# BICLab/Spike2Former

Measured on AMD Instinct MI355X. Metric: fwd+bwd images/sec, 512x512 T=4 ADE20K-150, higher is better.
Workload: dtype f32 (fp32-equivalent: bf16 hi+mid+lo split operands on bf16 MFMA, fp32 accumulate; spike maps stored as bf16, exact); 1 GPU; C2: 512x512 T=4 K=150 Meta-SpikeFormer [64, 128, 256, 360] + MaskFormer head, per-GPU batch 2; global_batch=2, parallelism=dp1, weights=random-init (name-seeded)

## Files before the change

include/s2f.h:

```cpp
#ifndef S2F_H
#define S2F_H

#include <stdint.h>

#ifdef __cplusplus
extern "C" {
#endif

#define S2F_OK 0
#define S2F_EINVAL (-1)
#define S2F_EALIGN (-2)
#define S2F_ELAUNCH (-3)

#define S2F_ABI_VERSION 52
#define S2F_STAT_SLOTS 256

int s2f_version(void);
const char* s2f_last_error(void);

void* s2f_event_create(void);
void s2f_event_destroy(void* event);
int s2f_time_next_call(void* start_event, void* stop_event);
int s2f_event_elapsed_us(void* start_event, void* stop_event, double* microseconds);

int64_t s2f_lif_mask_words(int64_t n);

int s2f_lif_fwd(const float* x, const float* v_in, void* y, float* v_out, uint64_t* mask, uint8_t* count_u8,
                uint64_t* stats, int64_t n, float vth, int D, int y_bf16, void* stream);

int s2f_lif_bwd(const float* gy, const float* gv_out, const uint64_t* mask, float* gx, int64_t n, float vth, int D,
                void* stream);
int s2f_lif_bwd_ports(const float* gy, const float* gy2, const float* gv_out, const uint64_t* mask, const float* skip, float* gx,
                      int64_t n, float vth, int D, void* stream);

int s2f_lif_leaky_fwd(const float* x, const float* v_in, void* y, float* v_out, uint64_t* mask, uint64_t* stats, int64_t n, float vth,
                      int D, float tau, int decay_input, int y_bf16, void* stream);
int s2f_lif_leaky_bwd(const float* gy, const float* gv_out, const uint64_t* mask, float* gx, float* gv_in, int64_t n, float vth, int D,
                      float tau, int decay_input, void* stream);

int s2f_sum2_lif_fwd(const float* x, const float* e, const float* pos, void* y_key, void* y_value, uint64_t* mask_key,
                     uint64_t* mask_value, int64_t TB, int64_t B, int64_t C, int64_t L, float vth, int D, int y_bf16,
                     void* stream);
int s2f_sum2_lif_bwd(const float* g_key, const float* g_value, const uint64_t* mask_key, const uint64_t* mask_value,
                     float* gx, int64_t n, int D, void* stream);
int s2f_sum2_lif_bwd_ex(const float* g_key, const float* g_value, const uint64_t* mask_key, const uint64_t* mask_value, float* gx,
                        float* gx_key, int64_t n, int D, void* stream);
int s2f_sum2_lif_bwd_ports(const float* g_key, const float* g_key2, const float* g_value, const float* g_value2,
// ... 136 lines not shown
                           float* bn_partials, int batch, int Mo, int Ki, int N, void* stream);
int s2f_bn_partials_finalize(const float* partials, int64_t P, const float* conv_bias, double* sums_out, int64_t N, int64_t C,
                             int64_t L, void* stream);
int s2f_bn_grouped_ok(int64_t N, int64_t C, int64_t L);
int s2f_bn_act_fwd_grouped(const float* z, const float* conv_bias, float* stat_out, float* running_mean, float* running_var,
                           const float* gamma, const float* beta, float* u_out, void* y_out, uint64_t* mask, int groups, int64_t N,
                           int64_t C, int64_t L, float momentum, float eps, float vth, int D, int y_bf16, void* stream);
int s2f_bn_act_bwd_grouped(const float* z, const float* conv_bias, const float* stat, const float* gamma, const float* g_u,
                           const float* g_y, const uint64_t* mask, float* gz, float* dgamma, float* dbeta, int groups, int64_t N,
                           int64_t C, int64_t L, float vth, int D, void* stream);
int s2f_bn_bwd_ports_ok(int64_t N, int64_t C, int64_t L, int training, int D);
int s2f_bn_act_bwd_ports(const float* z, const float* conv_bias, const float* stat, const float* gamma, const float* g_u,
                         const float* g_y, const float* g_y2, const float* g_v, const uint64_t* mask, double* sums_zeroed, float* gz,
                         float* g_residual, float* dgamma, float* dbeta, int64_t N, int64_t C, int64_t L, int training, float vth,
                         int D, void* stream);

int s2f_bn_act_bwd_split(const float* z, const float* conv_bias, const float* stat, const float* gamma, const float* g_u,
                         const float* g_y, const float* g_v, const uint64_t* mask, double* sums_zeroed, uint16_t* gz_split,
                         float* g_residual, float* dgamma, float* dbeta, int64_t N, int64_t C, int64_t L, int training,
                         float vth, int D, void* stream);
int s2f_pgemm_dx_split(const uint16_t* w_pack, const uint16_t* G_split, int64_t plane_stride, float* DX, int batch, int Mo,
                       int Ki, int N, int cfg, void* stream);
int s2f_spike_gemm_dw_bf16_split(const uint16_t* dY_split, int64_t plane_stride, const uint16_t* X, float* dW, int batch, int M,
                                 int K, int L, int accumulate, void* stream);
int s2f_spike_gemm_dw_grouped_split(const int64_t* jobs, int njobs, int bkv, void* stream);
int s2f_gemm_dw_general(const float* dY, int64_t dy_batch_stride, const float* X, int64_t x_batch_stride, float* dW, int batch,
                        int M, int K, int L, int accumulate, void* stream);
int s2f_gemm_dw_general_grouped(const int64_t* jobs, int njobs, void* stream);

int s2f_upsample2x_fwd(const float* x, float* y, int64_t planes, int h, int w, void* stream);
int s2f_upsample2x_sigmoid_fwd(const float* x, float* y, int64_t planes, int h, int w, void* stream);
int s2f_upsample2x_bwd(const float* gy, float* gx, int64_t planes, int h, int w, void* stream);
int s2f_upsample2x_bwd_add(const float* gy, const float* add, float* gx, int64_t planes, int h, int w, void* stream);

#define S2F_RESIZE_ALIGN_CORNERS 1
#define S2F_RESIZE_SIGMOID 2
#define S2F_RESIZE_FLIP_H 4
#define S2F_RESIZE_FLIP_V 8
int s2f_resize_fwd(const float* x, float* y, int64_t planes, int64_t plane_stride, int row_stride, int row0, int col0, int h, int w,
                   int H, int W, int flags, void* stream);
int s2f_resize_bwd_add(const float* gy, const float* add, float* gx, int64_t planes, int h, int w, int H, int W, int flags,
                       void* stream);
int s2f_seg_argmax(const float* x, int64_t* label, float* label_f, int K, int64_t HW, int sigmoid, float threshold, void* stream);
int s2f_seg_label(const float* x, int64_t* label, float* label_f, int K, int64_t plane_stride, int row_stride, int row0, int col0,
                  int h, int w, int H, int W, int flags, float threshold, void* stream);
int s2f_tta_accumulate(const float* x, float* acc, int K, int64_t plane_stride, int row_stride, int row0, int col0, int h, int w,
                       int H, int W, int flags, int first, void* stream);
int s2f_tta_finish(float* acc, int64_t* label, float* label_f, int K, int64_t HW, int n_views, float threshold, void* stream);

int s2f_slide_windows(const float* x, float* out, int B, int C, int H, int W, int crop_h, int crop_w, int stride_h, int stride_w,
                      int w0, int n, void* stream);
int s2f_slide_accumulate(const float* logits, float* preds, int B, int K, int H, int W, int crop_h, int crop_w, int stride_h,
                         int stride_w, int w0, int n, void* stream);

#define S2F_SEG_HIST_MAX_CLASSES 2048
#define S2F_SEG_PRED_I64 0
#define S2F_SEG_PRED_F32 1
#define S2F_SEG_LABEL_U8 0
#define S2F_SEG_LABEL_I64 1
#define S2F_SEG_REDUCE_ZERO_LABEL 1
int s2f_seg_hist(const void* pred, int pred_dtype, const void* label, int label_dtype, int64_t label_row_stride,
                 int64_t label_pixel_stride, int W, int64_t HW, int K, int ignore_index, int flags, int64_t* totals, void* stream);
#define S2F_SEG_CONF_LDS_BYTES 131072
#define S2F_SEG_CONF_GLOBAL 2
int s2f_seg_confusion(const void* pred, int pred_dtype, const void* label, int label_dtype, int64_t label_row_stride,
                      int64_t label_pixel_stride, int W, int64_t HW, int K, int ignore_index, int flags, int64_t* matrix, void* stream);
// ... 163 lines not shown
```

spike2former_amd/_lib.py:

```python
import ctypes
import os

import torch

_HERE = os.path.dirname(os.path.abspath(__file__))
LIB_PATH = os.environ.get("S2F_LIB") or os.path.join(_HERE, "libs2f_hip.so")

_p, _i, _i64, _f = ctypes.c_void_p, ctypes.c_int, ctypes.c_int64, ctypes.c_float

SIGNATURES = {
    "s2f_version": (_i, []),
    "s2f_last_error": (ctypes.c_char_p, []),
    "s2f_event_create": (_p, []),
    "s2f_event_destroy": (None, [_p]),
    "s2f_time_next_call": (_i, [_p, _p]),
    "s2f_event_elapsed_us": (_i, [_p, _p, ctypes.POINTER(ctypes.c_double)]),
    "s2f_lif_mask_words": (_i64, [_i64]),
    "s2f_lif_fwd": (_i, [_p, _p, _p, _p, _p, _p, _p, _i64, _f, _i, _i, _p]),
    "s2f_lif_bwd": (_i, [_p, _p, _p, _p, _i64, _f, _i, _p]),
    "s2f_lif_bwd_ports": (_i, [_p] * 6 + [_i64, _f, _i, _p]),
    "s2f_lif_leaky_fwd": (_i, [_p, _p, _p, _p, _p, _p, _i64, _f, _i, _f, _i, _i, _p]),
    "s2f_lif_leaky_bwd": (_i, [_p, _p, _p, _p, _p, _i64, _f, _i, _f, _i, _p]),
    "s2f_sum2_lif_fwd": (_i, [_p] * 7 + [_i64] * 4 + [_f, _i, _i, _p]),
    "s2f_sum2_lif_bwd": (_i, [_p] * 5 + [_i64, _i, _p]),
    "s2f_sum2_lif_bwd_ex": (_i, [_p] * 6 + [_i64, _i, _p]),
    "s2f_sum2_lif_bwd_ports": (_i, [_p] * 9 + [_i64, _i, _p]),
    "s2f_mask_loss_fwd": (_i, [_p] * 4 + [_i64, _i, _i, _f, _f, _p]),
    "s2f_mask_loss_bwd": (_i, [_p] * 5 + [_i64, _i, _i, _f, _f, _p]),
    "s2f_scale_affine_fwd": (_i, [_p] * 5 + [_i, _p]),
    "s2f_scale_affine_bwd": (_i, [_p] * 8 + [_i, _p]),
    "s2f_lif_seq_fwd": (_i, [_p, _p, _p, _p, _p, _p, _i, _i64, _f, _i, _p]),
    "s2f_lif_seq_bwd": (_i, [_p, _p, _p, _p, _p, _i, _i64, _f, _i, _p]),
    "s2f_bn_single_pass": (_i, [_i64] * 3),
    "s2f_bn_mask_words": (_i64, [_i64] * 3),
    "s2f_bn2_fused_ok": (_i, [_i64] * 3),
    "s2f_bn2_act_fwd": (_i, [_p] * 8 + [_f, _f] + [_p] * 5 + [_f, _f] + [_p] * 7 + [_i64] * 3 + [_f, _i, _i, _p]),
    "s2f_bn2_act_bwd": (_i, [_p] * 5 + [_f] + [_p] * 10 + [_i64] * 3 + [_f, _i, _p]),
    "s2f_bn_stats": (_i, [_p] * 3 + [_i64] * 3 + [_p]),
    "s2f_bn_act_fwd": (_i, [_p] * 16 + [_i64] * 3 + [_f, _f, _i, _f, _i, _i, _p]),
    "s2f_bn_act_bwd": (_i, [_p] * 13 + [_i64] * 3 + [_i, _f, _i, _p]),
    "s2f_bn_up_ok": (_i, [_i64] * 4 + [_i, _i]),
    "s2f_bn_act_up_fwd": (_i, [_p] * 16 + [_i64] * 4 + [_f, _f, _i, _f, _i, _i, _p]),
    "s2f_im2col": (_i, [_p, _p] + [_i] * 9 + [_p]),
    "s2f_col2im": (_i, [_p, _p] + [_i] * 8 + [_p]),
    "s2f_dwconv_fwd": (_i, [_p] * 4 + [_i] * 7 + [_p]),
    "s2f_dwconv_stats_slots": (_i64, [_i] * 3),
    "s2f_dwconv_fwd_stats": (_i, [_p] * 4 + [_i64] + [_i] * 5 + [_p]),
    "s2f_dwconv_bn_lif_fwd": (_i, [_p] * 7 + [_f] + [_p] * 3 + [_i] * 7 + [_f, _i, _p]),
    "s2f_dwconv_bwd_input": (_i, [_p] * 3 + [_i] * 6 + [_p]),
    "s2f_dwconv_bwd_weight": (_i, [_p] * 4 + [_i] * 8 + [_p]),
    "s2f_split_bf16x3": (_i, [_p, _p, _i, _i, _i, _i, _p]),
    "s2f_split_bf16x3_multi": (_i, [_p, _i, _i64, _p]),
    "s2f_spike_gemm_fwd": (_i, [_p] * 4 + [_i] * 7 + [_p]),
    "s2f_upsample2x_fwd": (_i, [_p, _p, _i64, _i, _i, _p]),
    "s2f_upsample2x_sigmoid_fwd": (_i, [_p, _p, _i64, _i, _i, _p]),
    "s2f_upsample2x_bwd": (_i, [_p, _p, _i64, _i, _i, _p]),
    "s2f_upsample2x_bwd_add": (_i, [_p, _p, _p, _i64, _i, _i, _p]),
    "s2f_resize_fwd": (_i, [_p, _p, _i64, _i64] + [_i] * 8 + [_p]),
    "s2f_resize_bwd_add": (_i, [_p, _p, _p, _i64] + [_i] * 5 + [_p]),
    "s2f_seg_argmax": (_i, [_p, _p, _p, _i, _i64, _i, _f, _p]),
    "s2f_seg_label": (_i, [_p, _p, _p, _i, _i64] + [_i] * 8 + [_f, _p]),
    "s2f_tta_accumulate": (_i, [_p, _p, _i, _i64] + [_i] * 9 + [_p]),
    "s2f_tta_finish": (_i, [_p, _p, _p, _i, _i64, _i, _f, _p]),
    "s2f_slide_windows": (_i, [_p, _p] + [_i] * 10 + [_p]),
    "s2f_slide_accumulate": (_i, [_p, _p] + [_i] * 10 + [_p]),
    "s2f_seg_hist": (_i, [_p, _i, _p, _i, _i64, _i64, _i, _i64, _i, _i, _i, _p, _p]),
    "s2f_seg_confusion": (_i, [_p, _i, _p, _i, _i64, _i64, _i, _i64, _i, _i, _i, _p, _p]),
    "s2f_seg_draw": (_i, [_p, _p, _i, _p, _i, _p, _i, ctypes.c_double, _i, _i, _i, _p, _p]),
    "s2f_aug_param_bytes": (_i, []),
    "s2f_aug_crop_stats": (_i, [_p, _i64, _p, _i, _i, _i, _i, _i, ctypes.c_double, _p, _p]),
    "s2f_aug_apply": (_i, [_p, _i64, _p, _p, _i, _i, _i] + [_f] * 6 + [_i, _f, _i, _i, _p, _p, _p]),
    "s2f_view_param_bytes": (_i, []),
    "s2f_test_views": (_i, [_p, _i64, _p, _i, _i, _i] + [_f] * 6 + [_i, _f, _p, _i64, _p]),
    "s2f_transpose_last2": (_i, [_p, _p, _i64, _i, _i, _p]),
    "s2f_transpose_last2_add": (_i, [_p, _p, _p, _i64, _i, _i, _p]),
    "s2f_sum_n": (_i, [_p, _i, _p, _i64, _p]),
    "s2f_transpose_scale_add_fwd": (_i, [_p, _p, _p, _p, _i64, _i, _i, _p]),
    "s2f_transpose_scale_add_bwd": (_i, [_p, _p, _p, _p, _p, _i64, _i, _i, _p]),
    "s2f_spike_conv3x3_fwd": (_i, [_p, _p, _p, _p] + [_i] * 8 + [_p]),
    "s2f_spike_conv3x3_dw": (_i, [_p, _p, _p] + [_i] * 6 + [_p]),
    "s2f_conv3x3_general": (_i, [_p, _p, _p] + [_i] * 7 + [_p]),
    "s2f_split_gemm": (_i, [_p, _i64, _i64, _i, _p, _i64, _i, _i64, _i, _p, _i64, _f, _i, _i, _i, _i, _i, _i, _p]),
    "s2f_spike_gemm_dw": (_i, [_p, _p, _p, _i, _i, _i, _i, _i, _i, _p]),
    "s2f_to_bf16_exact": (_i, [_p, _p, _i64, _p]),
    "s2f_spike_gemm_fwd_bf16": (_i, [_p] * 4 + [_i] * 7 + [_p]),
    "s2f_spike_conv3x3_fwd_bf16": (_i, [_p, _p, _p, _p] + [_i] * 8 + [_p]),
    "s2f_spike_gemm_dw_bf16": (_i, [_p, _p, _p, _i, _i, _i, _i, _i, _p]),
    "s2f_spike_gemm_fwd_bf16_ex": (_i, [_p, _i64, _p, _i64, _i, _i64, _p, _i64, _f, _p, _i, _i, _i, _i, _i, _i, _p]),
    "s2f_pgemm_nn_bf16_ex": (_i, [_p, _i64, _p, _i64, _i, _i64, _p, _i64, _f, _p, _i, _i, _i, _i, _p]),
    "s2f_spike_gemm_dw_grouped": (_i, [_p, _i, _i, _p]),
# ... 111 lines not shown
```

spike2former_amd/csrc/im2col.hip:

```cpp
#include "s2f_common.h"

namespace {

template <typename T>
struct Vec4;
template <>
struct Vec4<float> {
  typedef float4 type;
};
template <>
struct Vec4<unsigned short> {
  typedef uint2 type;
};

template <typename T, int S>
__global__ __launch_bounds__(256) void im2col_kernel(const T* __restrict__ x, T* __restrict__ cols, int C, int H, int W, int kh,
                                                     int kw, int stride_rt, int pad, int Ho, int Wo) {
  const int stride = S > 0 ? S : stride_rt;
  const int L = Ho * Wo, l0 = ((int)blockIdx.x * 256 + (int)threadIdx.x) * 4;
  if (l0 >= L) return;
  const int rowi = blockIdx.y, kk = kh * kw;
  const int c = rowi / kk, tap = rowi - c * kk;
  const int ky = tap / kw, kx = tap - ky * kw;
  const T* xp = x + ((int64_t)blockIdx.z * C + c) * (int64_t)H * W;
  T v[4];
  int oy = l0 / Wo, ox = l0 - oy * Wo;
#pragma unroll
  for (int o = 0; o < 4; ++o) {
    const int iy = oy * stride + ky - pad, ix = ox * stride + kx - pad;
    v[o] = (l0 + o < L && iy >= 0 && iy < H && ix >= 0 && ix < W) ? xp[(int64_t)iy * W + ix] : (T)0;
    if (++ox == Wo) ox = 0, ++oy;
  }
  T* cp = cols + ((int64_t)blockIdx.z * gridDim.y + rowi) * (int64_t)L + l0;
  if ((L & 3) == 0) {
    typename Vec4<T>::type pk;
    __builtin_memcpy(&pk, v, sizeof(pk));
    *reinterpret_cast<typename Vec4<T>::type*>(cp) = pk;
  } else {
#pragma unroll
    for (int o = 0; o < 4; ++o)
      if (l0 + o < L) cp[o] = v[o];
  }
}

template <int S>
__global__ __launch_bounds__(256) void col2im_kernel(const float* __restrict__ cols, float* __restrict__ gx, int64_t planes, int H,
                                                     int W, int kh, int kw, int stride_rt, int pad, int Ho, int Wo) {
  const int stride = S > 0 ? S : stride_rt;
  const int kk = kh * kw, W4 = (W + 3) >> 2;
  const int64_t L = (int64_t)Ho * Wo;
  const int cell = (int)blockIdx.x * 256 + (int)threadIdx.x;
  const int64_t nc = (int64_t)blockIdx.z * gridDim.y + blockIdx.y;
  if (cell >= H * W4 || nc >= planes) return;
  const int y = cell / W4, x0 = (cell - y * W4) * 4;
  const float* cp = cols + nc * kk * L;
  float acc[4] = {0.f, 0.f, 0.f, 0.f};
  for (int ky = 0; ky < kh; ++ky) {
    const int ty = y + pad - ky;
    if (ty < 0) break;
    const int oy = ty / stride;
    if (oy * stride != ty || oy >= Ho) continue;
    for (int kx = 0; kx < kw; ++kx) {
      const float* rowp = cp + (int64_t)(ky * kw + kx) * L + (int64_t)oy * Wo;
#pragma unroll
      for (int o = 0; o < 4; ++o) {
        const int tx = x0 + o + pad - kx;
        const int ox = tx / stride;
        if (tx >= 0 && ox * stride == tx && ox < Wo && x0 + o < W) acc[o] += rowp[ox];
      }
    }
  }
  float* gp = gx + (nc * H + y) * (int64_t)W + x0;
  if ((W & 3) == 0) {
    *reinterpret_cast<float4*>(gp) = make_float4(acc[0], acc[1], acc[2], acc[3]);
  } else {
#pragma unroll
// ... 1 lines not shown
      if (x0 + o < W) gp[o] = acc[o];
  }
}

int geometry(const char* who, int N, int C, int H, int W, int kh, int kw, int stride, int pad, int& Ho, int& Wo) {
  S2F_REQUIRE(N > 0 && C > 0 && H > 0 && W > 0 && kh > 0 && kw > 0 && stride > 0 && pad >= 0, S2F_EINVAL, "%s: bad geometry", who);
  Ho = (H + 2 * pad - kh) / stride + 1;
  Wo = (W + 2 * pad - kw) / stride + 1;
  S2F_REQUIRE(Ho > 0 && Wo > 0, S2F_EINVAL, "%s: empty output", who);
  S2F_REQUIRE((int64_t)C * kh * kw < 65536 && N < 65536 && (int64_t)N * C < ((int64_t)1 << 30) && (int64_t)H * W < ((int64_t)1 << 31) &&
                  (int64_t)Ho * Wo < ((int64_t)1 << 31),
              S2F_EINVAL, "%s: shape too large for the launch grid", who);
  return S2F_OK;
}

constexpr int kStrides[] = {1, 2, 0};
template <class F>
void for_stride(int stride, const F& launch) {
  s2f_dispatch<kStrides>([&](int sv) { return sv == stride || sv == 0; }, launch);
}

}

extern "C" int s2f_im2col(const void* x, void* cols, int N, int C, int H, int W, int kh, int kw, int stride, int pad, int x_bf16,
                          void* stream) {
  S2F_REQUIRE(x && cols, S2F_EINVAL, "s2f_im2col: null pointer");
  int Ho, Wo;
  int rc = geometry("s2f_im2col", N, C, H, W, kh, kw, stride, pad, Ho, Wo);
  if (rc) return rc;
  S2F_REQUIRE((((int64_t)Ho * Wo) & 3) != 0 || (reinterpret_cast<uintptr_t>(cols) & (x_bf16 ? 7u : 15u)) == 0, S2F_EALIGN,
              "s2f_im2col: cols must be 8-byte (bf16) / 16-byte (fp32) aligned");
  const dim3 grid((unsigned)((((int64_t)Ho * Wo + 3) / 4 + 255) / 256), (unsigned)(C * kh * kw), (unsigned)N);
  hipStream_t s = (hipStream_t)stream;
  for_stride(stride, [&](auto i) {
    s2f_dispatch_bool(x_bf16 != 0, [&](auto bf) {
      using T = std::conditional_t<bf.value, unsigned short, float>;
      hipLaunchKernelGGL((im2col_kernel<T, kStrides[i]>), grid, dim3(256), 0, s, reinterpret_cast<const T*>(x),
                         reinterpret_cast<T*>(cols), C, H, W, kh, kw, stride, pad, Ho, Wo);
    });
  });
  return s2f_check_launch("s2f_im2col");
}

extern "C" int s2f_col2im(const float* cols, float* gx, int N, int C, int H, int W, int kh, int kw, int stride, int pad,
                          void* stream) {
  S2F_REQUIRE(cols && gx, S2F_EINVAL, "s2f_col2im: null pointer");
  int Ho, Wo;
  int rc = geometry("s2f_col2im", N, C, H, W, kh, kw, stride, pad, Ho, Wo);
  if (rc) return rc;
  S2F_REQUIRE((W & 3) != 0 || s2f_aligned16(gx), S2F_EALIGN, "s2f_col2im: gx must be 16-byte aligned");
  const int64_t planes = (int64_t)N * C;
  const unsigned gy = (unsigned)(planes < 32768 ? planes : 32768);
  const dim3 grid((unsigned)(((int64_t)H * ((W + 3) / 4) + 255) / 256), gy, (unsigned)((planes + gy - 1) / gy));
  hipStream_t s = (hipStream_t)stream;
  for_stride(stride, [&](auto i) {
    hipLaunchKernelGGL(col2im_kernel<kStrides[i]>, grid, dim3(256), 0, s, cols, gx, planes, H, W, kh, kw, stride, pad, Ho, Wo);
  });
  return s2f_check_launch("s2f_col2im");
}
```

spike2former_amd/csrc/upsample.hip:

```cpp
#include "s2f_common.h"

#pragma clang fp contract(off)

namespace {

__device__ __forceinline__ void taps(int o, int in_size, int& i0, int& i1, float& l1) {
  float src = ((float)o + 0.5f) * 0.5f - 0.5f;
  if (src < 0.f) src = 0.f;
  i0 = (int)src;
  i1 = i0 + (i0 < in_size - 1 ? 1 : 0);
  l1 = src - (float)i0;
}

__global__ __launch_bounds__(256) void up2x_fwd_kernel(const float* __restrict__ x, float* __restrict__ y, int64_t planes,
                                                       int h, int w) {
  const int W = 2 * w, H = 2 * h;
  const int64_t quads_per_row = W / 4;
  const int64_t total = planes * H * quads_per_row;
  for (int64_t idx = (int64_t)blockIdx.x * blockDim.x + threadIdx.x; idx < total; idx += (int64_t)gridDim.x * blockDim.x) {
    const int q = (int)(idx % quads_per_row);
    const int64_t r = idx / quads_per_row;
    const int oy = (int)(r % H);
    const int64_t p = r / H;
    int y0, y1;
// ... 140 lines not shown
    const float wfirst = ix0 == 0 ? 1.f : 0.75f, wlast = ix0 + 4 == w ? 1.f : 0.75f;
    float acc0[4] = {0.f, 0.f, 0.f, 0.f}, acc1[4] = {0.f, 0.f, 0.f, 0.f};
#pragma unroll
    for (int rr = 0; rr < 6; ++rr) {
      const int oy = 2 * iy - 1 + rr;
      if (oy < 0 || oy >= H) continue;
      const float* row = base + (int64_t)oy * W + 8 * k;
      const float4 a = *reinterpret_cast<const float4*>(row), b = *reinterpret_cast<const float4*>(row + 4);
      const float left = k > 0 ? row[-1] : 0.f, right = k + 1 < qw ? row[8] : 0.f;
      float hx[4];
      hx[0] = (0.25f * left + wfirst * a.x) + (0.75f * a.y + 0.25f * a.z);
      hx[1] = (0.25f * a.y + 0.75f * a.z) + (0.75f * a.w + 0.25f * b.x);
      hx[2] = (0.25f * a.w + 0.75f * b.x) + (0.75f * b.y + 0.25f * b.z);
      hx[3] = (0.25f * b.y + 0.75f * b.z) + (wlast * b.w + 0.25f * right);
      float w0 = 0.f, w1 = 0.f;
      if (rr <= 3) w0 = (rr == 0 || rr == 3) ? 0.25f : ((rr == 1 && iy == 0) ? 1.f : 0.75f);
      if (rr >= 2) w1 = (rr == 2 || rr == 5) ? 0.25f : ((rr == 4 && iy + 2 == h) ? 1.f : 0.75f);
#pragma unroll
      for (int i = 0; i < 4; ++i) {
        acc0[i] += w0 * hx[i];
        acc1[i] += w1 * hx[i];
      }
    }
    float* o = gx + (p * h + iy) * w + ix0;
    if (add) {
      const float* q = add + (p * h + iy) * w + ix0;
      const float4 a0 = *reinterpret_cast<const float4*>(q), a1 = *reinterpret_cast<const float4*>(q + w);
      acc0[0] += a0.x, acc0[1] += a0.y, acc0[2] += a0.z, acc0[3] += a0.w;
      acc1[0] += a1.x, acc1[1] += a1.y, acc1[2] += a1.z, acc1[3] += a1.w;
    }
    *reinterpret_cast<float4*>(o) = make_float4(acc0[0], acc0[1], acc0[2], acc0[3]);
    *reinterpret_cast<float4*>(o + w) = make_float4(acc1[0], acc1[1], acc1[2], acc1[3]);
  }
}

struct MaskPix {
  float s, t, bce, pt, at;
};

__device__ __forceinline__ MaskPix mask_pix(float u, unsigned char tb, float alpha) {
  MaskPix m;
  m.t = tb ? 1.f : 0.f;
  const float e = __expf(-fabsf(u));
  const float inv = 1.f / (1.f + e);
  m.s = u >= 0.f ? inv : e * inv;
  m.bce = fmaxf(u, 0.f) - u * m.t + log1pf(e);
  m.pt = (1.f - m.s) * m.t + m.s * (1.f - m.t);
  m.at = alpha * m.t + (1.f - alpha) * (1.f - m.t);
  return m;
}

__global__ __launch_bounds__(256) void mask_loss_fwd_kernel(const float* __restrict__ pred, const unsigned char* __restrict__ tgt,
                                                            const int64_t* __restrict__ gt, float* __restrict__ sums, int h,
                                                            int w, float alpha, float gamma, int chunks) {
  const int W = 2 * w, H = 2 * h;
  const int p = blockIdx.y;
  const float* pp = pred + (int64_t)p * h * w;
  const unsigned char* tp = tgt + gt[p] * (int64_t)H * W;
  const int quads = W / 4;
  const int64_t total = (int64_t)H * quads;
  const int64_t per = (total + chunks - 1) / chunks;
  const int64_t beg = blockIdx.x * per, end = beg + per < total ? beg + per : total;
  float a = 0.f, b = 0.f, c = 0.f, f = 0.f;
  for (int64_t idx = beg + threadIdx.x; idx < end; idx += 256) {
    const int q = (int)(idx % quads), oy = (int)(idx / quads);
    int y0, y1;
// ... 90 lines not shown
  if ((w & 3) == 0 && s2f_aligned16(x))
    hipLaunchKernelGGL(up2x_fwd_block_kernel<false>, plane_grid((int64_t)h * (w / 4), planes), dim3(256), 0, (hipStream_t)stream, x, y,
                       planes, h, w);
  else
    hipLaunchKernelGGL(up2x_fwd_kernel, dim3(grid_for(planes * 2 * h * (2 * w / 4))), dim3(256), 0, (hipStream_t)stream, x, y,
                       planes, h, w);
  return s2f_check_launch("s2f_upsample2x_fwd");
}

extern "C" int s2f_upsample2x_sigmoid_fwd(const float* x, float* y, int64_t planes, int h, int w, void* stream) {
  S2F_REQUIRE(x && y, S2F_EINVAL, "s2f_upsample2x_sigmoid_fwd: null pointer");
  S2F_REQUIRE(planes > 0 && h > 0 && w > 0 && (w % 4) == 0, S2F_EINVAL, "s2f_upsample2x_sigmoid_fwd: needs w %% 4 == 0");
  S2F_REQUIRE(s2f_aligned16(x) && s2f_aligned16(y), S2F_EALIGN, "s2f_upsample2x_sigmoid_fwd: 16-byte alignment");
  hipLaunchKernelGGL(up2x_fwd_block_kernel<true>, plane_grid((int64_t)h * (w / 4), planes), dim3(256), 0, (hipStream_t)stream, x, y,
                     planes, h, w);
  return s2f_check_launch("s2f_upsample2x_sigmoid_fwd");
}

extern "C" int s2f_upsample2x_bwd_add(const float* gy, const float* add, float* gx, int64_t planes, int h, int w, void* stream) {
  S2F_REQUIRE(gy && gx, S2F_EINVAL, "s2f_upsample2x_bwd: null pointer");
  S2F_REQUIRE(planes > 0 && h > 0 && w > 0, S2F_EINVAL, "s2f_upsample2x_bwd: bad shape");
  if ((w & 3) == 0 && (h & 1) == 0 && s2f_aligned16(gy) && s2f_aligned16(gx) && s2f_aligned16(add))
    hipLaunchKernelGGL(up2x_bwd_block_kernel, plane_grid((int64_t)(h / 2) * (w / 4), planes), dim3(256), 0, (hipStream_t)stream,
                       gy, gx, planes, h, w, add);
  else
    hipLaunchKernelGGL(up2x_bwd_kernel, dim3(grid_for(planes * h * w)), dim3(256), 0, (hipStream_t)stream, gy, gx, planes, h, w, add);
  return s2f_check_launch("s2f_upsample2x_bwd");
}

extern "C" int s2f_upsample2x_bwd(const float* gy, float* gx, int64_t planes, int h, int w, void* stream) {
  return s2f_upsample2x_bwd_add(gy, nullptr, gx, planes, h, w, stream);
}

extern "C" int s2f_mask_loss_fwd(const float* pred, const uint8_t* tgt, const int64_t* gt_index, float* sums, int64_t P, int h,
                                 int w, float alpha, float gamma, void* stream) {
  if (P == 0) return S2F_OK;
  S2F_REQUIRE(pred && tgt && gt_index && sums, S2F_EINVAL, "s2f_mask_loss_fwd: null pointer");
  S2F_REQUIRE(P > 0 && P < 65536 && h > 0 && w > 0 && (w % 2) == 0, S2F_EINVAL, "s2f_mask_loss_fwd: need 0 < P < 65536, even w");
  S2F_REQUIRE((reinterpret_cast<uintptr_t>(tgt) & 3u) == 0, S2F_EALIGN, "s2f_mask_loss_fwd: targets must be 4-byte aligned");
  hipStream_t s = (hipStream_t)stream;
  if (s2f_zero_async(sums, sizeof(float) * 4 * (size_t)P, s) != S2F_OK) return s2f_check_launch("s2f_mask_loss_fwd memset");
  const int64_t total = (int64_t)2 * h * (2 * w / 4);
  int chunks = (int)((total + 256 * 8 - 1) / (256 * 8));
  if (chunks < 1) chunks = 1;
  hipLaunchKernelGGL(mask_loss_fwd_kernel, dim3(chunks, (unsigned)P), dim3(256), 0, s, pred, tgt, gt_index, sums, h, w, alpha,
                     gamma, chunks);
  return s2f_check_launch("s2f_mask_loss_fwd");
}

extern "C" int s2f_mask_loss_bwd(const float* pred, const uint8_t* tgt, const int64_t* gt_index, const float* g_sums, float* gup,
                                 int64_t P, int h, int w, float alpha, float gamma, void* stream) {
  if (P == 0) return S2F_OK;
  S2F_REQUIRE(pred && tgt && gt_index && g_sums && gup, S2F_EINVAL, "s2f_mask_loss_bwd: null pointer");
  S2F_REQUIRE(P > 0 && P < 65536 && h > 0 && w > 0 && (w % 2) == 0, S2F_EINVAL, "s2f_mask_loss_bwd: need 0 < P < 65536, even w");
  S2F_REQUIRE((reinterpret_cast<uintptr_t>(tgt) & 3u) == 0 && s2f_aligned16(gup), S2F_EALIGN,
              "s2f_mask_loss_bwd: targets 4-byte, gradient 16-byte aligned");
  const int64_t total = (int64_t)2 * h * (2 * w / 4);
  int chunks = (int)((total + 256 * 4 - 1) / (256 * 4));
  if (chunks < 1) chunks = 1;
  hipLaunchKernelGGL(mask_loss_bwd_kernel, dim3(chunks, (unsigned)P), dim3(256), 0, (hipStream_t)stream, pred, tgt, gt_index,
                     g_sums, gup, h, w, alpha, gamma, chunks);
  return s2f_check_launch("s2f_mask_loss_bwd");
}
```

spike2former_amd/ops/bn.py:

```python
import torch

from .config import cfg
from .core import *
from .resize import upsample_bilinear


class _BNAct(torch.autograd.Function):

    @staticmethod
    def forward(ctx, z, conv_bias, gamma, beta, residual, v_in, running_mean, running_var, nbt, training, momentum,
                eps, lif_on, want_pre, keep_v, D, vth, stats, bf16, partials=None, up_lo=None, up_skip=False, groups=1):
        _need_cuda(z, conv_bias, gamma, beta, residual, v_in, up_lo)
        ctx.groups = groups
        if groups > 1:
            return _BNAct._forward_siblings(ctx, z, conv_bias, gamma, beta, running_mean, running_var, momentum, eps, lif_on, want_pre,
                                            D, vth, bf16, groups, plain=(residual is None and v_in is None and nbt is None and training
                                                                         and not keep_v and stats is None and up_lo is None))
        up_in = up_lo
        z = z.contiguous()
        N, C = z.shape[0], z.shape[1]
        L = z.numel() // (N * C)
        dev = z.device
        stat = torch.empty(3 * C, dtype=torch.float32, device=dev)
        s = _stream()
# ... 91 lines not shown
        outs = [t if t is not None else z.new_empty(0) for t in (u, y, None)]
        ctx.mark_non_differentiable(border, ydata, tok2, through, *[o for o, t in zip(outs, (u, y, None)) if t is None])
        return tuple(outs) + (border, ydata, tok2, through)

    @staticmethod
    def backward(ctx, g_u, g_y, g_v, g_border, _g_ydata, g_y2, g_through=None):
        z, conv_bias, gamma, stat, mask = ctx.saved_tensors
        N, C, L, training, D, vth, has_res, has_bias = ctx.cfg

        def prep(g):
            return None if (g is None or g.numel() == 0) else g.contiguous()
        g_u, g_y, g_v, g_y2 = prep(g_u), prep(g_y), prep(g_v), prep(g_y2)
        if ctx.groups > 1:
            if g_u is None and g_y is None:
                return (None,) * 23
            G = ctx.groups
            gz = torch.empty_like(z)
            dgamma = torch.empty(G * C, dtype=torch.float32, device=z.device)
            dbeta = torch.empty(G * C, dtype=torch.float32, device=z.device)
            alg = 4 * z.numel() * (2 + (g_u is not None) + (g_y is not None))
            _time_next("bn_lif_bwd" if g_y is not None else "bn_bwd", alg)
            check(lib.s2f_bn_act_bwd_grouped(_ptr(z), _ptr(conv_bias), _ptr(stat), _ptr(gamma), _ptr(g_u), _ptr(g_y), _ptr(mask),
                                             _ptr(gz), _ptr(dgamma), _ptr(dbeta), G, N, C, L, vth, D, _stream()),
                  "s2f_bn_act_bwd_grouped")
            return (gz, None, dgamma, dbeta) + (None,) * 19
        if g_y is None:
            g_y, g_y2 = g_y2, None
        if g_y2 is not None and not lib.s2f_bn_bwd_ports_ok(N, C, L, int(training), D):
            g_y, g_y2 = g_y + g_y2, None
        if g_u is None and g_y is None and g_v is None:
            return (None,) * 20 + (g_through, None, None)
        dev = z.device
        gz = torch.empty_like(z)
        g_res = torch.empty_like(z) if ((has_res and ctx.needs_input_grad[4]) or (ctx.up is not None and ctx.needs_input_grad[20])) else None
        dgamma = torch.empty(C, dtype=torch.float32, device=dev)
        dbeta = torch.empty(C, dtype=torch.float32, device=dev)
        ws = None if (training and lib.s2f_bn_single_pass(N, C, L)) else _take_zeroed(2 * C, dev)
        alg = 4 * z.numel() * (2 + (g_u is not None) + (g_y is not None) + (g_res is not None))
        _time_next("bn_lif_bwd" if g_y is not None else "bn_bwd", alg, moved=alg + 4 * z.numel() * (g_y2 is not None))
        check(lib.s2f_bn_act_bwd_ports(_ptr(z), _ptr(conv_bias), _ptr(stat), _ptr(gamma), _ptr(g_u), _ptr(g_y), _ptr(g_y2), _ptr(g_v),
                                       _ptr(mask), _ptr(ws), _ptr(gz), _ptr(g_res), _ptr(dgamma), _ptr(dbeta), N, C, L,
                                       int(training), vth, D, _stream()), "s2f_bn_act_bwd_ports")
        g_bias = None
        if has_bias:
            g_bias = None if training else gamma * stat[C:2 * C] * dbeta
        if ctx.needs_input_grad[5]:
            raise RuntimeError("gradient w.r.t. the incoming membrane is not supported by the fused BN+LIF op")
        if ctx.up is not None:
            g_lo = g_through
            if g_res is not None:
                h, w = ctx.up
                g_lo = torch.empty(N, C, h, w, dtype=torch.float32, device=dev)
                check(lib.s2f_upsample2x_bwd_add(_ptr(g_res), _ptr(None if g_through is None else g_through.contiguous()), _ptr(g_lo),
                                                 N * C, h, w, _stream()), "s2f_upsample2x_bwd_add")
            return (gz, g_bias, dgamma, dbeta, None) + (None,) * 15 + (g_lo, None, None)
        return (gz, g_bias, dgamma, dbeta, g_res) + (None,) * 18


def _partial_slots(z):
    N, C = z.shape[0], z.shape[1]
    out = (int(lib.s2f_bn_partials_count(N, z.numel() // (N * C))),)
    if z.dim() == 4:
        out += (int(lib.s2f_dwconv_stats_slots(N, z.shape[2], z.shape[3])),)
    return out


def bn_up_ok(z, lo, training, D=8):
    if not (training and z.dim() == 4 and lo.dim() == 4 and z.is_cuda and lo.is_cuda and z.dtype == lo.dtype == torch.float32
            and z.numel() and lo.shape[:2] == z.shape[:2] and (2 * lo.shape[2], 2 * lo.shape[3]) == tuple(z.shape[2:])):
        return False
    return bool(lib.s2f_bn_up_ok(z.shape[0], z.shape[1], z.shape[2], z.shape[3], 1, D))


def bn_siblings_ok(z):
    return bool(z.dim() == 4 and 1 < z.shape[0] <= 4 and z.is_cuda and z.dtype == torch.float32 and z.numel()
                and lib.s2f_bn_grouped_ok(z.shape[1], z.shape[2], z.shape[3]))


def bn_act_siblings(z, conv_bias, gamma, beta, running_mean, running_var, momentum, eps, lif=False, want_pre=True, D=8, vth=1.0):
    bf16 = bool(lif) and spikes_bf16_ok(D) and z[0].numel() % 4 == 0
    u, y, _v, _border, ydata, _tok2, _thr = _BNAct.apply(z, conv_bias, gamma, beta, None, None, running_mean, running_var, None, True,
                                                         momentum, eps, lif, want_pre, False, D, vth, None, bf16, None, None, False,
                                                         int(z.shape[0]))
    if lif:
        y = Spikes(ydata, y) if bf16 else Spikes(y, None)
    return (u if want_pre else None), (y if lif else None)


def bn_act(z, conv_bias, gamma, beta, running_mean, running_var, nbt, training, momentum, eps, residual=None,
# ... 139 lines not shown
```

spike2former_amd/ops/config.py:

```python
import os


class Config:
    FIELDS = ("KERNEL_EVENTS", "GRAD_SINKS", "WGRAD_STREAM", "BRANCH_STREAMS", "LONG_STREAMS", "LONG_WHAT", "SPIKES_BF16",
              "SPIKE_GEMM_TERMS", "SPIKE_GEMM_ENABLED", "SPIKE_GEMM_CHECK", "CONV3X3_IMPLICIT", "CONV3X3_IMPLICIT_MIN_PIXELS",
              "CONV3X3_DX_IMPLICIT", "DEFER_DW", "DW_PIPE", "BN_PARTIALS", "BN_PARTIALS_SINGLE", "DENSE_GROUPED", "RESPLIT_IN_GRAPH",
              "FANOUT_PORTS", "GLUE_MODE", "STRICT_GLUE", "STRICT", "GENERAL_RESIZE")
    RUNTIME = ("KERNEL_EVENTS", "GRAD_SINKS", "WGRAD_STREAM", "BRANCH_STREAMS", "LONG_STREAMS")
    LAUNCH_FIELDS = ("DECODER_SIBLINGS", "DCN_CHANNEL_MAJOR")

    def __setattr__(self, name, value):
        if name not in self.FIELDS and name not in self.LAUNCH_FIELDS:
            raise AttributeError(f"ops.cfg has no switch {name!r} (the switches are ops.cfg.FIELDS)")
        object.__setattr__(self, name, value)

    def __init__(self):
        self.KERNEL_EVENTS = None
        self.GRAD_SINKS = None
        self.WGRAD_STREAM = None
        self.DEFER_DW = True
        self.BRANCH_STREAMS = None
        self.LONG_STREAMS = None
        self.LONG_WHAT = ("lat", "mf", "kv")
        self.SPIKES_BF16 = True
        self.SPIKE_GEMM_TERMS = 3
        self.SPIKE_GEMM_ENABLED = True
        self.CONV3X3_IMPLICIT = True
        self.CONV3X3_IMPLICIT_MIN_PIXELS = int(os.environ.get("S2F_CONV3_MIN_PIXELS", 32 * 32))
        self.CONV3X3_DX_IMPLICIT = True
        self.DW_PIPE = os.environ.get("S2F_DW_PIPE", "1") != "0"
        self.SPIKE_GEMM_CHECK = False
        self.BN_PARTIALS = os.environ.get("S2F_BN_PARTIALS", "1") != "0"
        self.BN_PARTIALS_SINGLE = os.environ.get("S2F_BN_PARTIALS_SINGLE", "0") != "0"
        self.DENSE_GROUPED = os.environ.get("S2F_DENSE_GROUPED", "1") != "0"
        self.RESPLIT_IN_GRAPH = True
        self.FANOUT_PORTS = os.environ.get("S2F_FANOUT_PORTS", "1") != "0"
        self.GLUE_MODE = os.environ.get("S2F_GLUE_MODE", "0") != "0"
        self.STRICT_GLUE = os.environ.get("S2F_STRICT_GLUE", "0") != "0"
        self.STRICT = os.environ.get("S2F_STRICT", "0") != "0"
        self.GENERAL_RESIZE = True
        self.DECODER_SIBLINGS = os.environ.get("S2F_DEC_SIBLINGS", "1") != "0"
        self.DCN_CHANNEL_MAJOR = os.environ.get("S2F_DCN_CM", "1") != "0"

    def snapshot(self):
        return {n: getattr(self, n) for n in self.FIELDS if n not in self.RUNTIME and n not in ("STRICT", "STRICT_GLUE")}

    def launch_snapshot(self):
        return dict(self.snapshot(), **{n: getattr(self, n) for n in self.LAUNCH_FIELDS})


cfg = Config()
```

Before: 58.25 images/s.

## Fuse LIF-mask gradient into upsample backward and add stride-2 row im2col

Adds a kernel that applies the LIF spike mask and 1/D scaling to the output gradients, stages the result in LDS, and performs the bilinear 2x upsample backward (plus optional add) in one pass. This lets the BN+LIF backward skip materializing the full-resolution g_res tensor when no membrane or u-gradient is needed, removing one write and one read of a large buffer. Separately, a stride-2 im2col kernel for 7x7/pad3 and 3x3/pad1 loads each input row once per (c,ky) and emits all kx taps, reducing redundant global reads. The fused path costs LDS capacity and needs alignment and shape preconditions.

```diff
diff --git a/include/s2f.h b/include/s2f.h
--- a/include/s2f.h
+++ b/include/s2f.h
@@ -12,7 +12,7 @@
 #define S2F_EALIGN (-2)
 #define S2F_ELAUNCH (-3)
 
-#define S2F_ABI_VERSION 52
+#define S2F_ABI_VERSION 53
 #define S2F_STAT_SLOTS 256
 
 int s2f_version(void);
@@ -215,6 +215,9 @@
 int s2f_upsample2x_sigmoid_fwd(const float* x, float* y, int64_t planes, int h, int w, void* stream);
 int s2f_upsample2x_bwd(const float* gy, float* gx, int64_t planes, int h, int w, void* stream);
 int s2f_upsample2x_bwd_add(const float* gy, const float* add, float* gx, int64_t planes, int h, int w, void* stream);
+int s2f_upsample2x_bwd_gu_ok(int64_t planes, int h, int w, int D);
+int s2f_upsample2x_bwd_gu(const float* g_y, const float* g_y2, const uint64_t* mask, const float* add, float* gx, int64_t planes,
+                          int h, int w, int D, void* stream);
 
 #define S2F_RESIZE_ALIGN_CORNERS 1
 #define S2F_RESIZE_SIGMOID 2
diff --git a/spike2former_amd/_lib.py b/spike2former_amd/_lib.py
--- a/spike2former_amd/_lib.py
+++ b/spike2former_amd/_lib.py
@@ -56,6 +56,8 @@
     "s2f_upsample2x_sigmoid_fwd": (_i, [_p, _p, _i64, _i, _i, _p]),
     "s2f_upsample2x_bwd": (_i, [_p, _p, _i64, _i, _i, _p]),
     "s2f_upsample2x_bwd_add": (_i, [_p, _p, _p, _i64, _i, _i, _p]),
+    "s2f_upsample2x_bwd_gu_ok": (_i, [_i64, _i, _i, _i]),
+    "s2f_upsample2x_bwd_gu": (_i, [_p] * 5 + [_i64, _i, _i, _i, _p]),
     "s2f_resize_fwd": (_i, [_p, _p, _i64, _i64] + [_i] * 8 + [_p]),
     "s2f_resize_bwd_add": (_i, [_p, _p, _p, _i64] + [_i] * 5 + [_p]),
     "s2f_seg_argmax": (_i, [_p, _p, _p, _i, _i64, _i, _f, _p]),
diff --git a/spike2former_amd/csrc/im2col.hip b/spike2former_amd/csrc/im2col.hip
--- a/spike2former_amd/csrc/im2col.hip
+++ b/spike2former_amd/csrc/im2col.hip
@@ -42,6 +42,45 @@
       if (l0 + o < L) cp[o] = v[o];
   }
 }
+
+template <typename T, int KW, int PAD>
+__global__ __launch_bounds__(256) void im2col_s2_rows_kernel(const T* __restrict__ x, T* __restrict__ cols, int C, int H, int W, int kh,
+                                                             int Ho, int Wo) {
+  constexpr int VE = 16 / (int)sizeof(T);
+  constexpr int NU = (VE + 6 + KW - 1 - PAD + 1 + VE - 1) / VE;
+  static_assert(PAD <= VE, "the first tap must lie in the first unit");
+  const int L = Ho * Wo, l0 = ((int)blockIdx.x * 256 + (int)threadIdx.x) * 4;
+  if (l0 >= L) return;
+  const int c = (int)blockIdx.y / kh, ky = (int)blockIdx.y - c * kh;
+  const int oy = l0 / Wo, ox0 = l0 - oy * Wo;
+  const int iy = 2 * oy + ky - PAD;
+  T buf[NU * VE];
+  const bool row_in = iy >= 0 && iy < H;
+  const T* rp = x + (((int64_t)blockIdx.z * C + c) * H + (row_in ? iy : 0)) * (int64_t)W;
+#pragma unroll
+  for (int u = 0; u < NU; ++u) {
+    const int ix = 2 * ox0 - VE + u * VE;
+    const bool in = row_in && ix >= 0 && ix < W;
+    uint4 v = *reinterpret_cast<const uint4*>(rp + (in ? ix : 0));
+    if (!in) v = make_uint4(0u, 0u, 0u, 0u);
+    __builtin_memcpy(&buf[u * VE], &v, sizeof(v));
+  }
+  T* cp = cols + (((int64_t)blockIdx.z * gridDim.y + blockIdx.y) * KW) * (int64_t)L + l0;
+#pragma unroll
+  for (int kx = 0; kx < KW; ++kx) {
+    T v[4];
+#pragma unroll
+    for (int o = 0; o < 4; ++o) v[o] = buf[VE + 2 * o + kx - PAD];
+    typename Vec4<T>::type pk;
+    __builtin_memcpy(&pk, v, sizeof(pk));
+    *reinterpret_cast<typename Vec4<T>::type*>(cp + (int64_t)kx * L) = pk;
+  }
+}
+
+struct S2Rows {
+  int kw, pad;
+};
+constexpr S2Rows kS2Rows[] = {{7, 3}, {3, 1}};
 
 template <int S>
 __global__ __launch_bounds__(256) void col2im_kernel(const float* __restrict__ cols, float* __restrict__ gx, int64_t planes, int H,
@@ -109,6 +148,16 @@
               "s2f_im2col: cols must be 8-byte (bf16) / 16-byte (fp32) aligned");
   const dim3 grid((unsigned)((((int64_t)Ho * Wo + 3) / 4 + 255) / 256), (unsigned)(C * kh * kw), (unsigned)N);
   hipStream_t s = (hipStream_t)stream;
+  if (stride == 2 && (Wo & 3) == 0 && W % (x_bf16 ? 8 : 4) == 0 && s2f_aligned16(x)) {
+    const bool taken = s2f_dispatch<kS2Rows>([&](const S2Rows& e) { return e.kw == kw && e.pad == pad; }, [&](auto i) {
+      s2f_dispatch_bool(x_bf16 != 0, [&](auto bf) {
+        using T = std::conditional_t<bf.value, unsigned short, float>;
+        hipLaunchKernelGGL((im2col_s2_rows_kernel<T, kS2Rows[i].kw, kS2Rows[i].pad>), dim3(grid.x, (unsigned)(C * kh), (unsigned)N),
+                           dim3(256), 0, s, reinterpret_cast<const T*>(x), reinterpret_cast<T*>(cols), C, H, W, kh, Ho, Wo);
+      });
+    });
+    if (taken) return s2f_check_launch("s2f_im2col");
+  }
   for_stride(stride, [&](auto i) {
     s2f_dispatch_bool(x_bf16 != 0, [&](auto bf) {
       using T = std::conditional_t<bf.value, unsigned short, float>;
diff --git a/spike2former_amd/csrc/upsample.hip b/spike2former_amd/csrc/upsample.hip
--- a/spike2former_amd/csrc/upsample.hip
+++ b/spike2former_amd/csrc/upsample.hip
@@ -196,6 +196,115 @@
     *reinterpret_cast<float4*>(o) = make_float4(acc0[0], acc0[1], acc0[2], acc0[3]);
     *reinterpret_cast<float4*>(o + w) = make_float4(acc1[0], acc1[1], acc1[2], acc1[3]);
   }
+}
+
+template <bool GY2>
+constexpr int kGuUnroll = GY2 ? 5 : 9;
+template <bool GY2>
+__global__ __launch_bounds__(256) void up2x_bwd_gu_kernel(const float* __restrict__ g_y, const float* __restrict__ g_y2,
+                                                          const uint64_t* __restrict__ mask, float* __restrict__ gx,
+                                                          int64_t planes, int h, int w,
+                                                          const float* __restrict__ add, int jb, float Df) {
+  extern __shared__ float4 up2x_gu_tile4[];
+  float* tile = reinterpret_cast<float*>(up2x_gu_tile4);
+  const int W = 2 * w, H = 2 * h;
+  const int qw = w / 4, qh = h / 2;
+  const int lane = threadIdx.x & 63, wv = __builtin_amdgcn_readfirstlane((int)(threadIdx.x >> 6));
+  const int jy0 = (int)blockIdx.x * jb, nj = min(jb, qh - jy0);
+  const int oy_lo = 4 * jy0 - 1;
+  const int r_first = max(oy_lo, 0), r_end = min(4 * (jy0 + nj) + 1, H);
+  const int jl = (int)threadIdx.x / qw, k = (int)threadIdx.x - jl * qw;
+  const bool worker = jl < nj;
+  const float inv_d = 1.0f / Df;
+  for (int64_t p = blockIdx.y; p < planes; p += gridDim.y) {
+    const int64_t pbase = p * H * W;
+    const int64_t e0 = pbase + (int64_t)r_first * W, e1 = pbase + (int64_t)r_end * W;
+    const int64_t lds0 = pbase + (int64_t)oy_lo * W;
+    const int64_t t_last = (e1 - 1) >> 8;
+    constexpr int U = kGuUnroll<GY2>;
+    for (int64_t t0 = (e0 >> 8) + wv; t0 <= t_last; t0 += 4 * U) {
+      float4 b[U], b2[U];
+      uint64_t mw[U][4];
+      bool act[U];
+#pragma unroll
+      for (int u = 0; u < U; ++u) {
+        const int64_t t = t0 + 4 * u, tc = t <= t_last ? t : t_last, e = t * 256 + lane * 4;
+        act[u] = t <= t_last && e >= e0 && e < e1;
+        const int64_t ec = act[u] ? e : e0;
+        b[u] = *reinterpret_cast<const float4*>(g_y + ec);
+        if (GY2) b2[u] = *reinterpret_cast<const float4*>(g_y2 + ec);
+#pragma unroll
+        for (int j = 0; j < 4; ++j) mw[u][j] = mask[tc * 4 + j];
+      }
+#pragma unroll
+      for (int u = 0; u < U; ++u) {
+        if (!act[u]) continue;
+        const float gy[4] = {b[u].x, b[u].y, b[u].z, b[u].w};
+        const float gy2[4] = {GY2 ? b2[u].x : 0.f, GY2 ? b2[u].y : 0.f, GY2 ? b2[u].z : 0.f, GY2 ? b2[u].w : 0.f};
+        float r[4];
+#pragma unroll
+        for (int j = 0; j < 4; ++j) {
+          const bool m = ((mw[u][j] >> lane) & 1ull) != 0;
+          const float gyv = GY2 ? gy[j] + gy2[j] : gy[j];
+          const float through = gyv * inv_d;
+          r[j] = m ? through : 0.f;
+        }
+        const int64_t e = (t0 + 4 * u) * 256 + lane * 4;
+        *reinterpret_cast<float4*>(tile + (e - lds0)) = make_float4(r[0], r[1], r[2], r[3]);
+      }
+    }
+    __syncthreads();
+    if (worker) {
+      const int iy = 2 * (jy0 + jl), ix0 = 4 * k;
+      float4 a0 = make_float4(0.f, 0.f, 0.f, 0.f), a1 = a0;
+      if (add) {
+        const float* q = add + (p * h + iy) * w + ix0;
+        a0 = *reinterpret_cast<const float4*>(q), a1 = *reinterpret_cast<const float4*>(q + w);
+      }
+      const float wfirst = ix0 == 0 ? 1.f : 0.75f, wlast = ix0 + 4 == w ? 1.f : 0.75f;
+      float acc0[4] = {0.f, 0.f, 0.f, 0.f}, acc1[4] = {0.f, 0.f, 0.f, 0.f};
+#pragma unroll
+      for (int rr = 0; rr < 6; ++rr) {
+        const int oy = 2 * iy - 1 + rr;
+        if (oy < 0 || oy >= H) continue;
+        const float* row = tile + (oy - oy_lo) * W + 8 * k;
+        const float4 a = *reinterpret_cast<const float4*>(row), b = *reinterpret_cast<const float4*>(row + 4);
+        const float left = k > 0 ? row[-1] : 0.f, right = k + 1 < qw ? row[8] : 0.f;
+        float hx[4];
+        hx[0] = (0.25f * left + wfirst * a.x) + (0.75f * a.y + 0.25f * a.z);
+        hx[1] = (0.25f * a.y + 0.75f * a.z) + (0.75f * a.w + 0.25f * b.x);
+        hx[2] = (0.25f * a.w + 0.75f * b.x) + (0.75f * b.y + 0.25f * b.z);
+        hx[3] = (0.25f * b.y + 0.75f * b.z) + (wlast * b.w + 0.25f * right);
+        float w0 = 0.f, w1 = 0.f;
+        if (rr <= 3) w0 = (rr == 0 || rr == 3) ? 0.25f : ((rr == 1 && iy == 0) ? 1.f : 0.75f);
+        if (rr >= 2) w1 = (rr == 2 || rr == 5) ? 0.25f : ((rr == 4 && iy + 2 == h) ? 1.f : 0.75f);
+#pragma unroll
+        for (int i = 0; i < 4; ++i) {
+          acc0[i] += w0 * hx[i];
+          acc1[i] += w1 * hx[i];
+        }
+      }
+      float* o = gx + (p * h + iy) * w + ix0;
+      if (add) {
+        acc0[0] += a0.x, acc0[1] += a0.y, acc0[2] += a0.z, acc0[3] += a0.w;
+        acc1[0] += a1.x, acc1[1] += a1.y, acc1[2] += a1.z, acc1[3] += a1.w;
+      }
+      *reinterpret_cast<float4*>(o) = make_float4(acc0[0], acc0[1], acc0[2], acc0[3]);
+      *reinterpret_cast<float4*>(o + w) = make_float4(acc1[0], acc1[1], acc1[2], acc1[3]);
+    }
+    __syncthreads();
+  }
+}
+
+inline int gu_band(int h, int w, size_t& lds) {
+  const int qw = w / 4, qh = h / 2;
+  int jb = qw >= 256 ? 1 : 256 / qw;
+  if (jb > qh) jb = qh;
+  lds = (size_t)(4 * jb + 2) * (size_t)(2 * w) * sizeof(float);
+  return jb;
+}
+inline bool gu_ok(int64_t planes, int h, int w, int D) {
+  return planes > 0 && h > 0 && w > 0 && (w & 3) == 0 && (h & 1) == 0 && w <= 1024 && h < (1 << 24) && D >= 1;
 }
 
 struct MaskPix {
@@ -352,6 +461,25 @@
   return s2f_upsample2x_bwd_add(gy, nullptr, gx, planes, h, w, stream);
 }
 
+extern "C" int s2f_upsample2x_bwd_gu_ok(int64_t planes, int h, int w, int D) { return gu_ok(planes, h, w, D) ? 1 : 0; }
+
+extern "C" int s2f_upsample2x_bwd_gu(const float* g_y, const float* g_y2, const uint64_t* mask, const float* add, float* gx,
+                                     int64_t planes, int h, int w, int D, void* stream) {
+  S2F_REQUIRE(g_y && mask && gx, S2F_EINVAL, "s2f_upsample2x_bwd_gu: null pointer");
+  S2F_REQUIRE(gu_ok(planes, h, w, D), S2F_EINVAL, "s2f_upsample2x_bwd_gu: needs w %% 4 == 0, w <= 1024, even h, D >= 1");
+  S2F_REQUIRE(s2f_aligned16(g_y) && s2f_aligned16(g_y2) && s2f_aligned16(add) && s2f_aligned16(gx) &&
+                  (reinterpret_cast<uintptr_t>(mask) & 7u) == 0,
+              S2F_EALIGN, "s2f_upsample2x_bwd_gu: gradients 16-byte, mask 8-byte aligned");
+  size_t lds;
+  const int jb = gu_band(h, w, lds);
+  const dim3 grid((unsigned)((h / 2 + jb - 1) / jb), (unsigned)(planes < 65535 ? planes : 65535));
+  s2f_dispatch_bool(g_y2 != nullptr, [&](auto y2) {
+    hipLaunchKernelGGL((up2x_bwd_gu_kernel<y2.value>), grid, dim3(256), lds, (hipStream_t)stream, g_y, g_y2, mask, gx, planes, h, w, add,
+                       jb, (float)D);
+  });
+  return s2f_check_launch("s2f_upsample2x_bwd_gu");
+}
+
 extern "C" int s2f_mask_loss_fwd(const float* pred, const uint8_t* tgt, const int64_t* gt_index, float* sums, int64_t P, int h,
                                  int w, float alpha, float gamma, void* stream) {
   if (P == 0) return S2F_OK;
diff --git a/spike2former_amd/ops/bn.py b/spike2former_amd/ops/bn.py
--- a/spike2former_amd/ops/bn.py
+++ b/spike2former_amd/ops/bn.py
@@ -147,7 +147,10 @@
             return (None,) * 20 + (g_through, None, None)
         dev = z.device
         gz = torch.empty_like(z)
-        g_res = torch.empty_like(z) if ((has_res and ctx.needs_input_grad[4]) or (ctx.up is not None and ctx.needs_input_grad[20])) else None
+        up_gu = bool(ctx.up is not None and ctx.needs_input_grad[20] and _up_bwd_gu_ok(ctx.up, N * C, D, g_u, g_y, g_y2, g_v, mask,
+                                                                                        g_through))
+        g_res = torch.empty_like(z) if ((has_res and ctx.needs_input_grad[4])
+                                        or (ctx.up is not None and ctx.needs_input_grad[20] and not up_gu)) else None
         dgamma = torch.empty(C, dtype=torch.float32, device=dev)
         dbeta = torch.empty(C, dtype=torch.float32, device=dev)
         ws = None if (training and lib.s2f_bn_single_pass(N, C, L)) else _take_zeroed(2 * C, dev)
@@ -163,13 +166,28 @@
             raise RuntimeError("gradient w.r.t. the incoming membrane is not supported by the fused BN+LIF op")
         if ctx.up is not None:
             g_lo = g_through
-            if g_res is not None:
-                h, w = ctx.up
+            h, w = ctx.up
+            if up_gu:
+                g_lo = torch.empty(N, C, h, w, dtype=torch.float32, device=dev)
+                check(lib.s2f_upsample2x_bwd_gu(_ptr(g_y), _ptr(g_y2), _ptr(mask),
+                                                _ptr(None if g_through is None else g_through.contiguous()), _ptr(g_lo), N * C, h, w, D,
+                                                _stream()), "s2f_upsample2x_bwd_gu")
+            elif g_res is not None:
                 g_lo = torch.empty(N, C, h, w, dtype=torch.float32, device=dev)
                 check(lib.s2f_upsample2x_bwd_add(_ptr(g_res), _ptr(None if g_through is None else g_through.contiguous()), _ptr(g_lo),
                                                  N * C, h, w, _stream()), "s2f_upsample2x_bwd_add")
             return (gz, g_bias, dgamma, dbeta, None) + (None,) * 15 + (g_lo, None, None)
         return (gz, g_bias, dgamma, dbeta, g_res) + (None,) * 18
+
+
+def _up_bwd_gu_ok(up, planes, D, g_u, g_y, g_y2, g_v, mask, g_through):
+    if not cfg.UP_BWD_GU or g_y is None or g_u is not None or g_v is not None or mask is None:
+        return False
+    if any(t is not None and (t.data_ptr() & 15 or not t.is_contiguous()) for t in (g_y, g_y2)):
+        return False
+    if g_through is not None and g_through.is_contiguous() and g_through.data_ptr() & 15:
+        return False
+    return bool(lib.s2f_upsample2x_bwd_gu_ok(planes, up[0], up[1], D))
 
 
 def _partial_slots(z):
diff --git a/spike2former_amd/ops/config.py b/spike2former_amd/ops/config.py
--- a/spike2former_amd/ops/config.py
+++ b/spike2former_amd/ops/config.py
@@ -7,7 +7,7 @@
               "CONV3X3_DX_IMPLICIT", "DEFER_DW", "DW_PIPE", "BN_PARTIALS", "BN_PARTIALS_SINGLE", "DENSE_GROUPED", "RESPLIT_IN_GRAPH",
               "FANOUT_PORTS", "GLUE_MODE", "STRICT_GLUE", "STRICT", "GENERAL_RESIZE")
     RUNTIME = ("KERNEL_EVENTS", "GRAD_SINKS", "WGRAD_STREAM", "BRANCH_STREAMS", "LONG_STREAMS")
-    LAUNCH_FIELDS = ("DECODER_SIBLINGS", "DCN_CHANNEL_MAJOR")
+    LAUNCH_FIELDS = ("DECODER_SIBLINGS", "DCN_CHANNEL_MAJOR", "UP_BWD_GU")
 
     def __setattr__(self, name, value):
         if name not in self.FIELDS and name not in self.LAUNCH_FIELDS:
@@ -41,6 +41,7 @@
         self.GENERAL_RESIZE = True
         self.DECODER_SIBLINGS = os.environ.get("S2F_DEC_SIBLINGS", "1") != "0"
         self.DCN_CHANNEL_MAJOR = os.environ.get("S2F_DCN_CM", "1") != "0"
+        self.UP_BWD_GU = os.environ.get("S2F_UP_BWD_GU", "1") != "0"
 
     def snapshot(self):
         return {n: getattr(self, n) for n in self.FIELDS if n not in self.RUNTIME and n not in ("STRICT", "STRICT_GLUE")}
```

New measurement: 58.81 images/s, median of 6. No clear change (+1.0%).
